# PFC-star/distributed_inference_demo

Measured on AMD Instinct MI355X. Metric: decode tokens/s, BLOOM pipeline, higher is better.
Workload: dtype bf16; 1 GPU; bloom-1b1 single stage on 1 MI355X, batch 1 decode after a 512-token prefill (BASELINE.json configs[1]); model=bloom-1b1, stages=1, batch=1, prompt=512, parallelism=pp1, weight_bytes=2130628608, weights=bf16

## Files before the change

### distributed_inference_demo_amd/build.py

```python
import hashlib
import os
import subprocess
import sys
from concurrent.futures import ThreadPoolExecutor

PKG = os.path.dirname(os.path.abspath(__file__))
ROOT = os.path.dirname(PKG)
CSRC = os.path.join(PKG, "csrc")
OBJ = os.path.join(PKG, "build")
LIB = os.path.join(PKG, "lib", "libbloomstage.so")
HIPCC = os.environ.get("HIPCC", "/opt/rocm/bin/hipcc")
ARCH = "gfx950"

SOURCES = ["kernels.hip", "attn_prefill.hip", "kv_int8.hip", "stage.hip", "codec.cpp", "safetensors.cpp"]
EXTRA = {"attn_prefill.hip": ["-mllvm", "-amdgpu-mfma-vgpr-form=1"]}
HEADERS = ["common.h", "kernels.h", "attn_merge.h", "safetensors.h"]
STAMP = os.path.join(OBJ, "build_id")
CFLAGS = ["-O3", "-std=c++17", "-fPIC", f"--offload-arch={ARCH}", "-Wall", "-Wno-unused-function",
          "-Wno-unused-variable", "-Wno-unused-result", "-Wno-unused-value", f"-I{os.path.join(ROOT, 'include')}"]


def _mtime(p):
    return os.path.getmtime(p) if os.path.exists(p) else 0.0


def source_hash() -> str:
    h = hashlib.sha256()
    for path in [os.path.join(CSRC, f) for f in SOURCES + HEADERS] + [os.path.join(ROOT, "include", "bloomstage.h")]:
        with open(path, "rb") as f:
            h.update(os.path.basename(path).encode() + b"\0" + f.read())
    return h.hexdigest()


def build(force: bool = False, verbose: bool = False) -> str:
    os.makedirs(OBJ, exist_ok=True)
    os.makedirs(os.path.dirname(LIB), exist_ok=True)
    bid = source_hash()
    old = open(STAMP).read().strip() if os.path.exists(STAMP) else ""
    restamp = old != bid
    hdr_t = max([_mtime(os.path.join(CSRC, h)) for h in HEADERS] + [_mtime(os.path.join(ROOT, "include", "bloomstage.h"))])
    jobs = []
    objs = []
    for src in SOURCES:
        sp = os.path.join(CSRC, src)
        op = os.path.join(OBJ, src + ".o")
        objs.append(op)
        if force or (restamp and src == "stage.hip") or _mtime(op) < max(_mtime(sp), hdr_t):
            flags = list(CFLAGS)
# ... 29 lines not shown
```

### distributed_inference_demo_amd/csrc/kernels.hip

```cpp
#include <array>
#include <cstdio>
#include <cstring>
#include <vector>
#include "common.h"
#include "kernels.h"
#include "attn_merge.h"

__device__ __forceinline__ __amdgpu_buffer_rsrc_t attn_rsrc(const void* p) {
  return __builtin_amdgcn_make_buffer_rsrc(const_cast<void*>(p), (short)0, (int)0xFFFFFFFF, 0x00020000);
}

#include <algorithm>
#include <cstdlib>

__device__ __forceinline__ uint64_t d_sm64(uint64_t x) {
  x += 0x9E3779B97F4A7C15ull;
  x = (x ^ (x >> 30)) * 0xBF58476D1CE4E5B9ull;
  x = (x ^ (x >> 27)) * 0x94D049BB133111EBull;
  return x ^ (x >> 31);
}
__device__ __forceinline__ uint32_t d_lb32(uint32_t x) {
  x ^= x >> 16; x *= 0x7feb352du; x ^= x >> 15; x *= 0x846ca68bu; x ^= x >> 16;
  return x;
}
// ... 120 lines not shown
  if constexpr (KIND == EPI_QKV) {
    v += to_f32(((const T*)e.bias)[n]);
    const int three = 3 * e.head_dim;
    const int head = n / three, r = n - head * three, which = r / e.head_dim, d = r - which * e.head_dim;
    if (which == 0) {
      ((T*)e.q_out)[(size_t)m * e.hidden + head * e.head_dim + d] = from_f32<T>(v);
    } else {
      const int b = m / e.seq, t = m - b * e.seq;
      const int past = e.past_dev ? e.past_dev[b] : e.past;
      const size_t idx = (((size_t)(e.slot + b) * e.n_head + head) * e.max_ctx + past + t) * e.head_dim + d;
      T* c = (T*)(which == 1 ? e.k_cache : e.v_cache);
      c[idx] = from_f32<T>(v);
    }
  } else if constexpr (KIND == EPI_RESID) {
    const size_t i = (size_t)m * e.ldo + n;
    e.out_f32[i] = (v + to_f32(((const T*)e.bias)[n])) + e.resid[i];
  } else if constexpr (KIND == EPI_GELU) {
    ((T*)e.out_act)[(size_t)m * e.ldo + n] = from_f32<T>(gelu_bloom(v + to_f32(((const T*)e.bias)[n])));
  }
}

struct EpiPre {
  uint32_t bias_bits;
  float resid;
  int past;
};

template <typename T>
__device__ __forceinline__ float bias_value(uint32_t bits) {
  if constexpr (sizeof(T) == 2) return __uint_as_float(bits << 16);
  else return __uint_as_float(bits);
}

template <typename T>
__device__ __forceinline__ EpiPre epi_prefetch(const Epi& e, int m, int n, bool valid) {
  EpiPre p{0u, 0.f, 0};
  if (e.kind == EPI_ARGMAX) return p;
  const int nn = valid ? n : 0, mm = valid ? m : 0;
  if constexpr (sizeof(T) == 2) p.bias_bits = ((const unsigned short*)e.bias)[nn];
  else p.bias_bits = ((const uint32_t*)e.bias)[nn];
  if (e.kind == EPI_RESID) p.resid = e.resid[(size_t)mm * e.ldo + nn];
  if (e.kind == EPI_QKV) p.past = e.past_dev ? e.past_dev[mm / e.seq] : e.past;
  return p;
}

template <typename T, int KIND>
__device__ __forceinline__ void epi_store_pre(const Epi& e, int m, int n, float v, const EpiPre& p) {
  if (e.col_scale) v *= e.col_scale[n];
  const float bias = bias_value<T>(p.bias_bits);
  if constexpr (KIND == EPI_QKV) {
    v += bias;
    const int three = 3 * e.head_dim;
    const int head = n / three, r = n - head * three, which = r / e.head_dim, d = r - which * e.head_dim;
    if (which == 0) {
      ((T*)e.q_out)[(size_t)m * e.hidden + head * e.head_dim + d] = from_f32<T>(v);
    } else {
      const int b = m / e.seq, t = m - b * e.seq;
      const size_t idx = (((size_t)(e.slot + b) * e.n_head + head) * e.max_ctx + p.past + t) * e.head_dim + d;
      T* c = (T*)(which == 1 ? e.k_cache : e.v_cache);
      c[idx] = from_f32<T>(v);
    }
  } else if constexpr (KIND == EPI_RESID) {
    e.out_f32[(size_t)m * e.ldo + n] = (v + bias) + p.resid;
  } else if constexpr (KIND == EPI_GELU) {
    ((T*)e.out_act)[(size_t)m * e.ldo + n] = from_f32<T>(gelu_bloom(v + bias));
  }
}

template <typename T, int K>
__device__ __forceinline__ void epi_apply(const Epi& ep, int m, int n, float v, bool valid, int ntiles) {
  if constexpr (K == EPI_ARGMAX) argmax_tile16(ep, m, n, v, valid, ntiles);
  else if (valid) epi_store<T, K>(ep, m, n, v);
}

template <int V> struct EpiKindC { static constexpr int value = V; };

template <typename F>
__device__ __forceinline__ void epi_dispatch(int kind, F&& f) {
  switch (kind) {
    case EPI_QKV: f(EpiKindC<EPI_QKV>{}); break;
    case EPI_RESID: f(EpiKindC<EPI_RESID>{}); break;
    case EPI_GELU: f(EpiKindC<EPI_GELU>{}); break;
    default: f(EpiKindC<EPI_ARGMAX>{}); break;
  }
}

struct LnArgs {
  const float* x;
  int row_stride, row_offset;
  const bf16* gamma;
  const bf16* beta;
// ... 134 lines not shown
#pragma unroll
    for (int u = 0; u < U; u++) {
      const bool live = s + u < s1;
#pragma unroll
      for (int mt = 0; mt < MT; mt++)
        acc[mt] = __builtin_amdgcn_mfma_f32_16x16x32_bf16(a[u], live ? b[mt][u] : zero8, acc[mt], 0, 0, 0);
    }
    if (more) {
#pragma unroll
      for (int u = 0; u < U; u++) a[u] = an[u];
    }
  }
  if constexpr (LN) __syncthreads();
#pragma unroll
  for (int mt = 0; mt < MT; mt++)
#pragma unroll
    for (int i = 0; i < 4; i++) red[w][mt * 16 + r][4 * g + i] = acc[mt][i];
  __syncthreads();
  const int ntiles = (N + 15) >> 4;
  epi_dispatch(ep.kind, [&](auto kc) {
    constexpr int EK = decltype(kc)::value;
    for (int t = threadIdx.x; t < MT * 256; t += WAVES * 64) {
      const int ml = t >> 4, nl = t & 15;
      float v = 0.f;
#pragma unroll
      for (int ww = 0; ww < WAVES; ww++) v += red[ww][ml][nl];
      const int n = n0 + nl;
      epi_apply<bf16, EK>(ep, ml, n, v, ml < M && n < N, ntiles);
    }
  });
}


template <int MM>
__device__ __forceinline__ void ln_rows_load(const LnArgs& ln, int M, int K, float4 (&xv)[MM][4], float (&c)[MM],
                                             uint2 (&gb)[4][2]) {
#pragma unroll
  for (int i = 0; i < 4; i++) {
    const int k = threadIdx.x * 4 + i * 1024;
    gb[i][0] = k < K ? *reinterpret_cast<const uint2*>(ln.gamma + k) : make_uint2(0u, 0u);
    gb[i][1] = k < K ? *reinterpret_cast<const uint2*>(ln.beta + k) : make_uint2(0u, 0u);
  }
#pragma unroll
  for (int m = 0; m < MM; m++) {
    const float* xr = ln.x + ((size_t)min(m, M - 1) * ln.row_stride + ln.row_offset) * K;
    c[m] = xr[0];
#pragma unroll
    for (int i = 0; i < 4; i++) {
      const int k = threadIdx.x * 4 + i * 1024;
      xv[m][i] = k < K ? *reinterpret_cast<const float4*>(xr + k) : make_float4(0.f, 0.f, 0.f, 0.f);
    }
  }
}

template <int MM>
__device__ __forceinline__ void ln_rows_finish(const LnArgs& ln, int M, int K, float4 (&xv)[MM][4],
                                               const float (&c)[MM], const uint2 (&gb)[4][2], bf16* xs,
                                               float* scratch) {
  const int lane = threadIdx.x & 63, w = threadIdx.x >> 6;
  const bool active = threadIdx.x < 256;
  float s1[MM], s2[MM];
#pragma unroll
  for (int m = 0; m < MM; m++) {
    float a1 = 0.f, a2 = 0.f;
#pragma unroll
    for (int i = 0; i < 4; i++) {
      if (threadIdx.x * 4 + i * 1024 < K) {
        const float d0 = xv[m][i].x - c[m], d1 = xv[m][i].y - c[m], d2 = xv[m][i].z - c[m], d3 = xv[m][i].w - c[m];
        a1 += (d0 + d1) + (d2 + d3);
        a2 += (d0 * d0 + d1 * d1) + (d2 * d2 + d3 * d3);
      }
    }
    s1[m] = wave_sum(a1);
    s2[m] = wave_sum(a2);
  }
  if (lane == 0 && active) {
#pragma unroll
    for (int m = 0; m < MM; m++) {
      scratch[w * 8 + m] = s1[m];
      scratch[32 + w * 8 + m] = s2[m];
    }
  }
  __syncthreads();
  float mean[MM], rstd[MM];
  const float invk = 1.0f / (float)K;
// ... 119 lines not shown
      for (int i = 0; i < 4; i++) {
        if (active && (int)threadIdx.x * 4 + i * 1024 < K) {
          if (pass == 0) a += (v[m][i].x + v[m][i].y) + (v[m][i].z + v[m][i].w);
          else {
            const float d0 = v[m][i].x - mean[m], d1 = v[m][i].y - mean[m], d2 = v[m][i].z - mean[m], d3 = v[m][i].w - mean[m];
            a += (d0 * d0 + d1 * d1) + (d2 * d2 + d3 * d3);
          }
        }
      }
      a = wave_sum(a);
      if (lane == 0 && active) scratch[pass * 32 + w * 8 + m] = a;
    }
    __syncthreads();
#pragma unroll
    for (int m = 0; m < MM; m++) {
      const float t = ((scratch[pass * 32 + m] + scratch[pass * 32 + 8 + m]) +
                       (scratch[pass * 32 + 16 + m] + scratch[pass * 32 + 24 + m])) * invk;
      if (pass == 0) mean[m] = t;
      else rstd[m] = 1.0f / sqrtf(t + eps);
    }
  }
  __syncthreads();
}

__device__ __forceinline__ void bf16x4_to_f32(const uint2 raw, float4& o) {
  o = make_float4(__uint_as_float(raw.x << 16), __uint_as_float(raw.x & 0xFFFF0000u),
                  __uint_as_float(raw.y << 16), __uint_as_float(raw.y & 0xFFFF0000u));
}

template <int MM>
__device__ __forceinline__ void emb_rows_prefetch(const LnArgs& ln, int M, int K, int (&id)[MM], uint2 (&egb)[4][2],
                                                  uint2 (&gb)[4][2]) {
#pragma unroll
  for (int m = 0; m < MM; m++) id[m] = ln.ids[min(m, M - 1)];
#pragma unroll
  for (int i = 0; i < 4; i++) {
    const int k = min((int)threadIdx.x * 4 + i * 1024, K - 4);
    egb[i][0] = *reinterpret_cast<const uint2*>(ln.emb_g + k);
    egb[i][1] = *reinterpret_cast<const uint2*>(ln.emb_b + k);
    gb[i][0] = *reinterpret_cast<const uint2*>(ln.gamma + k);
    gb[i][1] = *reinterpret_cast<const uint2*>(ln.beta + k);
  }
}

template <int MM>
__device__ __forceinline__ void emb_rows_finish(const LnArgs& ln, int M, int K, const int (&id)[MM],
                                                const uint2 (&egb)[4][2], const uint2 (&gb)[4][2], bf16* xs,
                                                float* scratch) {
  float4 v[MM][4];
#pragma unroll
  for (int m = 0; m < MM; m++) {
    const bf16* row = ln.wemb + (size_t)id[m] * K;
#pragma unroll
    for (int i = 0; i < 4; i++) {
      const int k = min((int)threadIdx.x * 4 + i * 1024, K - 4);
      bf16x4_to_f32(*reinterpret_cast<const uint2*>(row + k), v[m][i]);
    }
  }
  float mean[MM], rstd[MM];
  ln_stats_256<MM>(v, K, ln.eps, scratch, mean, rstd);
  const bool active = threadIdx.x < 256;
#pragma unroll
  for (int i = 0; i < 4; i++) {
    float4 g, b;
    bf16x4_to_f32(egb[i][0], g);
    bf16x4_to_f32(egb[i][1], b);
    const int k = (int)threadIdx.x * 4 + i * 1024;
// ... 4 lines not shown
      v[m][i].z = (v[m][i].z - mean[m]) * rstd[m] * g.z + b.z;
      v[m][i].w = (v[m][i].w - mean[m]) * rstd[m] * g.w + b.w;
      if (blockIdx.x == 0 && active && k < K && m < M) *reinterpret_cast<float4*>(ln.x_out + (size_t)m * K + k) = v[m][i];
    }
  }
  ln_stats_256<MM>(v, K, ln.eps, scratch, mean, rstd);
#pragma unroll
  for (int i = 0; i < 4; i++) {
    const int k = (int)threadIdx.x * 4 + i * 1024;
    if (active && k < K) {
      float4 g, b;
      bf16x4_to_f32(gb[i][0], g);
      bf16x4_to_f32(gb[i][1], b);
#pragma unroll
      for (int m = 0; m < MM; m++) {
        if (m < M) {
          typedef __bf16 bf16x4 __attribute__((ext_vector_type(4)));
          bf16x4 o;
          o[0] = (bf16)((v[m][i].x - mean[m]) * rstd[m] * g.x + b.x);
          o[1] = (bf16)((v[m][i].y - mean[m]) * rstd[m] * g.y + b.y);
          o[2] = (bf16)((v[m][i].z - mean[m]) * rstd[m] * g.z + b.z);
          o[3] = (bf16)((v[m][i].w - mean[m]) * rstd[m] * g.w + b.w);
          *reinterpret_cast<bf16x4*>(xs + (size_t)m * K + k) = o;
        }
      }
    }
  }
  __syncthreads();
}

template <int R, int MM, int U, int XM, int FL = 0, bool SYNC = false>
__device__ __forceinline__ void gemv_rows_block(const bf16* __restrict__ W, const bf16* __restrict__ X, const LnArgs& ln,
                                                const AttnParts& pa, int M, int N, int K, const Epi& ep, int bid,
                                                char* smem, unsigned* wait, unsigned target) {
  if constexpr (!SYNC) wait = nullptr;
  constexpr bool LN = XM == X_LN;
  BS_STAMP(0);
  float* scratch = reinterpret_cast<float*>(smem);
  bf16* xs = reinterpret_cast<bf16*>(smem + 256);
  const int lane = threadIdx.x & 63, w = threadIdx.x >> 6, nw = blockDim.x >> 6;
  const int n0 = (bid * nw + w) * R;
  const bf16* wr[R];
#pragma unroll
  for (int r = 0; r < R; r++) wr[r] = W + (size_t)min(n0 + r, N - 1) * K;
  const int er = lane / MM, em = lane % MM;
  const EpiPre pre = epi_prefetch<bf16>(ep, em, n0 + er, lane < R * MM && em < M && n0 + er < N);
  float4 xv[LN ? MM : 1][4];
  float xc[LN ? MM : 1];
  uint2 gb[4][2];
  if constexpr (LN) {
    if (threadIdx.x < 256) ln_rows_load<MM>(ln, M, K, xv, xc, gb);
  }
  int eid[XM == X_EMB ? MM : 1];
  uint2 egb[4][2];
  if constexpr (XM == X_EMB) emb_rows_prefetch<MM>(ln, M, K, eid, egb, gb);
  const int kq = K >> 2, ngroups = M * kq;
  PartsRegs pr[XM == X_PARTS ? kPartsPre : 1];
  auto pld1 = [wait](const float* p, size_t i) {
    if (wait) return __uint_as_float(__builtin_amdgcn_raw_buffer_load_b32(attn_rsrc(p), (uint32_t)(i * 4), 0, 16));
    return p[i];
  };
  auto pld4 = [wait](const float* p, size_t i) {
    if (wait)
      return __builtin_bit_cast(float4, __builtin_amdgcn_raw_buffer_load_b128(attn_rsrc(p), (uint32_t)(i * 4), 0, 16));
    return *reinterpret_cast<const float4*>(p + i);
  };
  if constexpr (XM == X_PARTS) {
    if (!wait) {
#pragma unroll
      for (int it = 0; it < kPartsPre; it++) {
        const int g = min((int)threadIdx.x + it * (int)blockDim.x, ngroups - 1);
        attn_parts_load(pa, g / kq, (g % kq) * 4, pld1, pld4, pr[it]);
      }
    }
  }
  bf16x8 wv[U][R];
#pragma unroll
  for (int u = 0; u < U; u++) {
    const int k = min(u * 512 + lane * 8, K - 8);
#pragma unroll
    for (int r = 0; r < R; r++) wv[u][r] = wload<!(FL & 1)>(wr[r] + k);
  }
  const bf16* xg;
  int xstride;
  if constexpr (LN) {
    ln_rows_finish<MM>(ln, M, K, xv, xc, gb, xs, scratch);
    xg = xs; xstride = K;
  } else if constexpr (XM == X_EMB) {
    emb_rows_finish<MM>(ln, M, K, eid, egb, gb, xs, scratch);
    xg = xs; xstride = K;
  } else if constexpr (XM == X_PARTS) {
    if (wait) {
      if (threadIdx.x == 0) {
        unsigned spins = 0;
        while (__builtin_amdgcn_raw_buffer_load_b32(attn_rsrc(wait), 0, 0, 16) < target) {
          __builtin_amdgcn_s_sleep(2);
          if (++spins > (1u << 22)) {
            __builtin_amdgcn_raw_buffer_store_b32(1u, attn_rsrc(wait), 8, 0, 16);
            break;
          }
        }
      }
      __syncthreads();
#pragma unroll
      for (int it = 0; it < kPartsPre; it++) {
        const int g = min((int)threadIdx.x + it * (int)blockDim.x, ngroups - 1);
        attn_parts_load(pa, g / kq, (g % kq) * 4, pld1, pld4, pr[it]);
      }
    }
    auto put = [&](int g, const PartsRegs& r) {
      float o[4];
      attn_parts_combine(pa.nsplit, r, o);
      typedef __bf16 bf16x4 __attribute__((ext_vector_type(4)));
      bf16x4 v;
#pragma unroll
      for (int j = 0; j < 4; j++) v[j] = (bf16)o[j];
      *reinterpret_cast<bf16x4*>(xs + (size_t)(g / kq) * K + (g % kq) * 4) = v;
    };
#pragma unroll
    for (int it = 0; it < kPartsPre; it++) {
      const int g = threadIdx.x + it * blockDim.x;
      if (g < ngroups) put(g, pr[it]);
    }
    for (int g = threadIdx.x + kPartsPre * blockDim.x; g < ngroups; g += blockDim.x) {
      PartsRegs r;
      attn_parts_load(pa, g / kq, (g % kq) * 4, pld1, pld4, r);
      put(g, r);
    }
    __syncthreads();
    xg = xs; xstride = K;
  } else {
    xg = X; xstride = K;
  }
  BS_STAMP(1);
  float acc[R][MM];
#pragma unroll
  for (int r = 0; r < R; r++)
#pragma unroll
    for (int m = 0; m < MM; m++) acc[r][m] = 0.f;
  const bf16x8 zero8 = (bf16x8){0, 0, 0, 0, 0, 0, 0, 0};
  for (int kb = 0; kb < K; kb += 512 * U) {
    if (kb) {
#pragma unroll
      for (int u = 0; u < U; u++) {
        const int k = min(kb + u * 512 + lane * 8, K - 8);
#pragma unroll
        for (int r = 0; r < R; r++) wv[u][r] = wload<!(FL & 1)>(wr[r] + k);
      }
    }
#pragma unroll
    for (int u = 0; u < U; u++) {
      const int kk = kb + u * 512 + lane * 8;
      const bool live = kk < K;
      const int k = min(kk, K - 8);
#pragma unroll
      for (int m = 0; m < MM; m++) {
        bf16x8 xv;
// ... 18 lines not shown
      if (lane == 0) {
#pragma unroll
        for (int r = 0; r < R; r++)
#pragma unroll
          for (int m = 0; m < MM; m++) tv[(w * R + r) * MM + m] = acc[r][m];
      }
      __syncthreads();
      if (threadIdx.x < 64) {
        const int col = threadIdx.x & 15, m = threadIdx.x >> 4;
        const int n = bid * 16 + col;
        const float v = m < MM ? tv[col * MM + (m < MM ? m : 0)] : 0.f;
        argmax_tile16(ep, m, n, v, m < M && n < N, (N + 15) >> 4);
      }
    } else {
      if (lane < R * MM) {
        float v = 0.f;
#pragma unroll
        for (int r = 0; r < R; r++)
#pragma unroll
          for (int m = 0; m < MM; m++) v = (lane == r * MM + m) ? acc[r][m] : v;
        const int n = n0 + er;
        if constexpr (FL & 4) {
          if (v == 12345.f) ep.keys[0] = 1;
        } else if (em < M && n < N) {
          epi_store_pre<bf16, EK>(ep, em, n, v, pre);
        }
      }
    }
  });
  BS_STAMP(3);
}

template <int R, int MM, int U, int XM, int FL = 0, int LB = 256>
__global__ __launch_bounds__(LB) void gemv_rows_kernel(const bf16* __restrict__ W, const bf16* __restrict__ X,
                                                         LnArgs ln, AttnParts pa, int M, int N, int K, Epi ep) {
  extern __shared__ __attribute__((aligned(16))) char smem[];
  gemv_rows_block<R, MM, U, XM, FL>(W, X, ln, pa, M, N, K, ep, blockIdx.x, smem, nullptr, 0u);
}

__device__ __forceinline__ void q8x16_to_bf16(const u32x4v raw, bf16x8& lo, bf16x8& hi) {
  const uint32_t v[4] = {raw.x ^ 0x80808080u, raw.y ^ 0x80808080u, raw.z ^ 0x80808080u, raw.w ^ 0x80808080u};
#pragma unroll
  for (int i = 0; i < 2; i++) {
    bf16x8& o = i ? hi : lo;
    const uint32_t a = v[2 * i], b = v[2 * i + 1];
    o[0] = (bf16)((float)(a & 0xFF) - 128.f); o[1] = (bf16)((float)((a >> 8) & 0xFF) - 128.f);
    o[2] = (bf16)((float)((a >> 16) & 0xFF) - 128.f); o[3] = (bf16)((float)(a >> 24) - 128.f);
    o[4] = (bf16)((float)(b & 0xFF) - 128.f); o[5] = (bf16)((float)((b >> 8) & 0xFF) - 128.f);
    o[6] = (bf16)((float)((b >> 16) & 0xFF) - 128.f); o[7] = (bf16)((float)(b >> 24) - 128.f);
  }
}

template <int T, int MT, int WAVES>
__device__ __forceinline__ void tiles_epilogue(const f32x4 (&acc)[T][MT], float* red, int M, int N, int n0,
                                               const Epi& ep) {
  constexpr int RS = MT * 16 + 1;
  const int lane = threadIdx.x & 63, w = threadIdx.x >> 6;
  const int r = lane & 15, g = lane >> 4;
  const int KS = gridDim.y, ks = blockIdx.y;
  float* rw = red + (size_t)w * (T * 16) * RS;
#pragma unroll
  for (int t = 0; t < T; t++)
#pragma unroll
    for (int mt = 0; mt < MT; mt++)
#pragma unroll
      for (int i = 0; i < 4; i++) rw[(t * 16 + 4 * g + i) * RS + mt * 16 + r] = acc[t][mt][i];
  __syncthreads();
  const int ntiles = (N + 15) >> 4;
  constexpr int TOTAL = T * 16 * MT * 16, NTH = WAVES * 64;
  constexpr int ITER = (TOTAL + NTH - 1) / NTH;
// ... 1133 lines not shown
    Ws[ty][tx] = wr[k0 + tx];
    __syncthreads();
#pragma unroll
    for (int kk = 0; kk < 16; kk++) acc += Xs[ty][kk] * Ws[tx][kk];
    __syncthreads();
  }
  const int m = m0 + ty, n = n0 + tx;
  epi_dispatch(ep.kind, [&](auto kc) {
    epi_apply<float, decltype(kc)::value>(ep, m, n, acc, m < M && n < N, (N + 15) >> 4);
  });
}

template <int WAVES, int MT, bool LN>
static void gemv_launch(const bf16* X, const LnArgs& ln, const bf16* W, int M, int N, int K, const Epi& ep,
                        hipStream_t s) {
  size_t shm = sizeof(float) * WAVES * MT * 16 * 17;
  if (LN) shm += (size_t)M * K * sizeof(bf16);
  gemv_mfma_kernel<WAVES, MT, 4, LN, 0, 0><<<(N + 15) / 16, WAVES * 64, shm, s>>>(W, X, ln, M, N, K, ep);
}

static int gemv_waves(int N, int K) {
  const int ntiles = (N + 15) / 16, ksteps = K / 32;
  int waves = 4;
  while (waves < 16 && ntiles * waves < 2048 && waves * 2 <= ksteps) waves *= 2;
  return waves;
}

template <int R, int MM, int XM, int U = 2, int FL = 0>
static void gemv_rows_launch(const bf16* X, const LnArgs& ln, const AttnParts& pa, const bf16* W, int M, int N,
                             int K, const Epi& ep, hipStream_t s, int waves = 4) {
  const size_t shm = 256 + (XM != X_PLAIN ? (size_t)M * K * sizeof(bf16) : 0);
  const int blocks = (N + waves * R - 1) / (waves * R);
  if (waves <= 4) {
    gemv_rows_kernel<R, MM, U, XM, FL, 256><<<blocks, waves * 64, shm, s>>>(W, X, ln, pa, M, N, K, ep);
  } else if constexpr (MM <= 2) {
    gemv_rows_kernel<R, MM, U, XM, FL, 1024><<<blocks, waves * 64, shm, s>>>(W, X, ln, pa, M, N, K, ep);
  }
}

static void rows_geometry(int N, int K, int M, int r_default, int* R, int* waves) {
  if (M > 2) { *R = r_default; *waves = 4; return; }
  const int rows_cu = (N + 255) / 256;
  int r = K <= 2048 ? 2 : 1;
  while ((rows_cu + r - 1) / r > 16 && r < 4) r *= 2;
  if ((rows_cu + r - 1) / r < 4) r = 1;
  *R = r;
  *waves = std::max(4, std::min(16, (rows_cu + r - 1) / r));
}

static void rows_plan(int XM, int M, int N, int K, int* R, int* waves, int* U) {
  const bool LN = XM == X_LN || XM == X_EMB;
  const int R0 = !LN ? (K <= 2048 ? 2 : 1) : (N >= 12288 ? 4 : (N >= 2048 ? 2 : 1));
  rows_geometry(N, K, M, R0, R, waves);
  const int cpr = K / 512;
  int u = (K % 512) ? 4 : (cpr <= 3 || cpr == 5 || cpr == 8 || cpr == 12) ? cpr
        : (cpr % 12 == 0 ? 12 : (cpr % 8 == 0 ? 8 : (cpr % 5 == 0 ? 5 : 4)));
  if (*waves > 4) {
    const int cap = (XM == X_PLAIN ? 12 : 8) / (M == 1 ? 1 : 2);
    while (*R * u > cap) u = (u % 2 == 0) ? u / 2 : (u > 4 ? 4 : u - 1);
  }
  *U = u;
}

template <int XM>
static bool gemv_rows_dispatch(const bf16* x, const LnArgs& ln, const AttnParts& pa, const bf16* w, int M, int N,
                               int K, const Epi& ep, hipStream_t s) {
  if (M > 4 || (K % 8) != 0 || K < 8 || (XM != X_PLAIN && K > 4096)) return false;
  if ((XM == X_PLAIN || XM == X_LN) && ep.kind != EPI_ARGMAX && tiles_take(M, K) && (K % 64) == 0) return false;
  if (XM == X_PLAIN && M > 2 && ep.kind != EPI_ARGMAX && (size_t)N * K > (size_t)16 << 20) return false;
// ... 810 lines not shown
            for (int i = 0; i < 4; i++) {
              xf[i] = f2{__uint_as_float(a0[i] << 16), __uint_as_float(a0[i] & 0xFFFF0000u)};
              xf[4 + i] = f2{__uint_as_float(a1[i] << 16), __uint_as_float(a1[i] & 0xFFFF0000u)};
            }
#pragma unroll
            for (int i = 0; i < 8; i++) xs[m] += xf[i];
#pragma unroll
            for (int r = 0; r < R; r++)
#pragma unroll
              for (int i = 0; i < 8; i++) acc[r][m] = __builtin_elementwise_fma(xf[i], wf[r][i], acc[r][m]);
          }
        }
      }
    }
  }
  float mine = 0.f;
#pragma unroll
  for (int r = 0; r < R; r++)
#pragma unroll
    for (int m = 0; m < MM; m++) {
      if (m < M) {
        const float t = wave_sum((acc[r][m].x + acc[r][m].y) - 128.f * (xs[m].x + xs[m].y));
        if (lane == r * MM + m) mine = t;
      }
    }
  const int r = lane / MM, m = lane - r * MM;
  if (lane < R * MM && m < M && n0 + r < N) epi_store<bf16, KIND>(ep, m, n0 + r, mine);
}

template <int R, int MM, bool LN, int CW, bool XL = false, int UQ = 2, bool PARTS = false, bool WIDE = false>
__global__ __launch_bounds__(WIDE ? 1024 : 256) void gemv_q8_kernel(const int8_t* __restrict__ Q, const float* __restrict__ scale,
                                                      const bf16* __restrict__ X, LnArgs ln, AttnParts pa, int M,
                                                      int N, int K, Epi ep) {
  epi_dispatch(ep.kind, [&](auto kc) {
    if constexpr (decltype(kc)::value != EPI_ARGMAX)
      gemv_q8_body<R, MM, LN, decltype(kc)::value, CW, XL, UQ, PARTS>(Q, scale, X, ln, pa, M, N, K, ep);
  });
}

template <int R, int MM, bool LN = false, bool PARTS = false>
static void gemv_q8_launch(const int8_t* Q, const float* scale, const bf16* X, const LnArgs& ln, int M, int N, int K,
                           const Epi& ep, hipStream_t s, const AttnParts& pa = AttnParts{}) {
  const size_t shm = (LN || PARTS) ? (size_t)M * K * sizeof(bf16) : 0;
  const int blocks = (N + 4 * R - 1) / (4 * R);
  const int steps = (K + 1023) / 1024;
  const int uq = (size_t)N * K > (12u << 20) ? 1 : min(steps <= 2 ? 2 : steps <= 4 ? 4 : steps <= 6 ? 6 : 8, R >= 4 ? 4 : 8);
  const bool wide_xl = (size_t)M * K * sizeof(bf16) <= 65536;
  if constexpr (MM == 1 && R <= 2) {
    int rr = 0, waves = 0;
    rows_geometry(N, K, M, R, &rr, &waves);
    if ((size_t)N * K <= (32u << 20) && rr <= 2 && waves >= 4 && uq <= 6) {
      auto go = [&](auto rc) {
        constexpr int RW = decltype(rc)::value;
        const int wb = (N + waves * RW - 1) / (waves * RW);
        const dim3 g(wb), t(waves * 64);
        if constexpr (!LN && !PARTS) {
          if (wide_xl) {
            const size_t shx = (size_t)M * K * sizeof(bf16);
            if (uq == 1) gemv_q8_kernel<RW, 1, false, 16, true, 1, false, true><<<g, t, shx, s>>>(Q, scale, X, ln, pa, M, N, K, ep);
            else if (uq <= 2) gemv_q8_kernel<RW, 1, false, 16, true, 2, false, true><<<g, t, shx, s>>>(Q, scale, X, ln, pa, M, N, K, ep);
            else if (uq <= 4) gemv_q8_kernel<RW, 1, false, 16, true, 4, false, true><<<g, t, shx, s>>>(Q, scale, X, ln, pa, M, N, K, ep);
            else gemv_q8_kernel<RW, 1, false, 16, true, 6, false, true><<<g, t, shx, s>>>(Q, scale, X, ln, pa, M, N, K, ep);
            return;
          }
        }
        if (uq == 1) gemv_q8_kernel<RW, 1, LN, 16, false, 1, PARTS, true><<<g, t, shm, s>>>(Q, scale, X, ln, pa, M, N, K, ep);
// ... 120 lines not shown
template <int MM, int U, int R>
__global__ __launch_bounds__(1024) void gemv_head_screen_kernel(const int8_t* __restrict__ Q, const float* __restrict__ scale,
                                                           const float* __restrict__ cb, LnArgs ln, int M, int ntiles,
                                                           int K, float2* __restrict__ hilo, float* __restrict__ rnorm) {
  typedef float f2 __attribute__((ext_vector_type(2)));
  extern __shared__ __attribute__((aligned(16))) char smem[];
  float* scratch = reinterpret_cast<float*>(smem);
  bf16* xs = reinterpret_cast<bf16*>(smem + 256);
  const int lane = threadIdx.x & 63, nw = blockDim.x >> 6;
  const int w = __builtin_amdgcn_readfirstlane(threadIdx.x >> 6);
  const int t0 = (int)((long long)blockIdx.x * ntiles / gridDim.x);
  const int t1 = (int)((long long)(blockIdx.x + 1) * ntiles / gridDim.x);
  constexpr int G = 16 / R;
  const int steps = (K + 512 * U - 1) / (512 * U), gs = G * steps;
  const int nunits = max((t1 - t0 - w + nw - 1) / nw, 0) * gs;
  typedef unsigned int u32x2v __attribute__((ext_vector_type(2)));
  struct Buf { u32x2v wv[U][R]; float sc[R], cc[R]; };
  auto issue = [&](int i, Buf& b) {
    const int ti = i / gs, rem = i - ti * gs, g = rem / steps, kb = rem - g * steps;
    const int n0 = (t0 + w + ti * nw) * 16 + g * R;
#pragma unroll
    for (int u = 0; u < U; u++) {
      const int col = min((kb * U + u) * 512 + lane * 8, K - 8);
#pragma unroll
      for (int r = 0; r < R; r++)
        b.wv[u][r] = __builtin_nontemporal_load(reinterpret_cast<const u32x2v*>(Q + (size_t)(n0 + r) * K + col));
    }
#pragma unroll
    for (int r = 0; r < R; r++) { b.sc[r] = scale[n0 + r]; b.cc[r] = cb[n0 + r]; }
  };
  float4 xv[MM][4];
  float xc[MM];
  uint2 gb[4][2];
  if (threadIdx.x < 256) ln_rows_load<MM>(ln, M, K, xv, xc, gb);
  Buf b0{}, b1{}, b2{};
  if (nunits > 0) issue(0, b0);
  if (nunits > 1) issue(1, b1);
  if (threadIdx.x < 8) xs[(size_t)M * K + threadIdx.x] = (bf16)0.f;
  ln_rows_finish<MM>(ln, M, K, xv, xc, gb, xs, scratch);
  float rm[MM];
#pragma unroll
  for (int m = 0; m < MM; m++) {
    float a = 0.f;
    for (int k = lane * 8; k < K; k += 512) {
      float v[8];
      load8(xs + (size_t)min(m, M - 1) * K + k, v);
#pragma unroll
      for (int j = 0; j < 8; j++) a = fmaf(v[j], v[j], a);
    }
    rm[m] = sqrtf(wave_sum(a)) * (1.0f + 0x1p-10f);
    if (blockIdx.x == 0 && threadIdx.x == 0 && m < M) rnorm[m] = rm[m];
    rm[m] *= 1.0f + 0x1p-20f;
  }
  float hi[MM], lo[MM], chk[MM];
  f2 acc[R][MM];
#pragma unroll
  for (int m = 0; m < MM; m++) {
    hi[m] = -INFINITY; lo[m] = -INFINITY; chk[m] = 0.f;
#pragma unroll
    for (int r = 0; r < R; r++) acc[r][m] = f2{0.f, 0.f};
  }
  auto compute = [&](int i, const Buf& cur) {
    const int ti = i / gs, rem = i - ti * gs, g = rem / steps, kb = rem - g * steps;
#pragma unroll
    for (int u = 0; u < U; u++) {
      const int kk = (kb * U + u) * 512 + lane * 8;
      f2 xf[MM][4];
// ... 83 lines not shown
  }
  L = wave_max(L);
  bad = __any(bad);
  if ((threadIdx.x & 63) == 0) { shl[threadIdx.x >> 6] = L; shb[threadIdx.x >> 6] = bad; }
  if (threadIdx.x == 0) cnt = 0;
  __syncthreads();
  L = shl[0]; bad = shb[0];
  for (int j = 1; j < 16; j++) { L = fmaxf(L, shl[j]); bad |= shb[j]; }
  bool all = bad || !(fabsf(L) < INFINITY) || !(fabsf(r) < INFINITY);
  if (!all) {
    if (fits) {
#pragma unroll
      for (int j = 0; j < kSelPer; j++) {
        const int i = threadIdx.x + j * 1024;
        if (i < ntiles && v[j].x >= L) li[atomicAdd(&cnt, 1)] = i;
      }
    } else {
      for (int i = threadIdx.x; i < ntiles; i += 1024)
        if (hl[i].x >= L) li[atomicAdd(&cnt, 1)] = i;
    }
    __syncthreads();
    all = cnt == 0;
  }
  if (all)
    for (int i = threadIdx.x; i < ntiles; i += 1024) li[i] = i;
  if (threadIdx.x == 0) { count[m] = all ? ntiles : cnt; lstar[m] = L; }
}

template <int MM, int U>
__global__ __launch_bounds__(256) void head_rescore_kernel(const bf16* __restrict__ W, LnArgs ln, int M, int N, int K,
                                                           Epi ep, const int* __restrict__ list,
                                                           const int* __restrict__ count, int ntiles) {
  extern __shared__ __attribute__((aligned(16))) char smem[];
  bool first = true;
  for (int m = 0; m < M; m++) {
    const int c = min(max(count[m], 0), ntiles);
    for (int i = blockIdx.x; i < c; i += gridDim.x) {
      const int tile = min(max(list[(size_t)m * ntiles + i], 0), ntiles - 1);
      if (!first) __syncthreads();
      first = false;
      gemv_rows_block<4, MM, U, X_LN>(W, nullptr, ln, AttnParts{}, M, N, K, ep, tile, smem, nullptr, 0u);
    }
  }
}

__global__ __launch_bounds__(1024) void head_screen_finalize_kernel(const unsigned long long* __restrict__ keys, int ntiles,
                                                                    const int* __restrict__ list,
                                                                    const int* __restrict__ count, int* tokens,
                                                                    int* past_adv, int seq) {
  __shared__ unsigned long long sh[17];
  const int m = blockIdx.x;
  const int c = min(max(count[m], 0), ntiles);
  unsigned long long best = 0;
  for (int i = threadIdx.x; i < c; i += 1024) {
    const int tile = min(max(list[(size_t)m * ntiles + i], 0), ntiles - 1);
    const unsigned long long k = keys[(size_t)m * ntiles + tile];
    best = k > best ? k : best;
  }
  best = block_max_u64(best, sh);
  if (threadIdx.x == 0) {
    if (tokens) tokens[m] = (int)(0xFFFFFFFFu - (uint32_t)(best & 0xFFFFFFFFull));
    if (past_adv) past_adv[m] += seq;
  }
}

bool head_screen_supported(int M, int K) { return M >= 1 && M <= 2 && K % 32 == 0 && K >= 32 && K <= 4096; }

template <int MM>
static void head_screen_launch(const HeadScreen& hs, const LnArgs& ln, int M, int ntiles, int K, int grid, hipStream_t s) {
  const size_t shm = 256 + (size_t)M * K * sizeof(bf16) + 16;
  float2* hl = reinterpret_cast<float2*>(hs.hilo);
  const int cpr = (K + 511) / 512;
#define HS_GO(UU, RR) gemv_head_screen_kernel<MM, UU, RR><<<grid, 1024, shm, s>>>(hs.Q, hs.scale, hs.cb, ln, M, ntiles, K, hl, hs.rnorm)
  if (cpr == 1) HS_GO(1, 4);
// ... 35 lines not shown
```

Baseline: 1224 tokens/s.

## Preload kernel arguments into SGPRs and reorder early loads in GEMV kernels

Enables kernarg preloading for kernels.hip and moves the most-used scalar arguments (LN pointers, strides, wave count) to the front of the gemv_rows kernel signature. Inline-asm pins force those values into SGPRs early. A lane_zero trick turns uniform scalar loads into vector loads so they issue alongside the other global loads, and the gamma/beta loads are reordered. The aim is to cut kernel-prologue latency in the small per-token decode kernels, at the cost of fragile asm constraints and compiler-flag dependence.

```diff
diff --git a/distributed_inference_demo_amd/build.py b/distributed_inference_demo_amd/build.py
--- a/distributed_inference_demo_amd/build.py
+++ b/distributed_inference_demo_amd/build.py
@@ -13,7 +13,8 @@
 ARCH = "gfx950"
 
 SOURCES = ["kernels.hip", "attn_prefill.hip", "kv_int8.hip", "stage.hip", "codec.cpp", "safetensors.cpp"]
-EXTRA = {"attn_prefill.hip": ["-mllvm", "-amdgpu-mfma-vgpr-form=1"]}
+EXTRA = {"attn_prefill.hip": ["-mllvm", "-amdgpu-mfma-vgpr-form=1"],
+         "kernels.hip": ["-mllvm", "-amdgpu-kernarg-preload-count=16"]}
 HEADERS = ["common.h", "kernels.h", "attn_merge.h", "safetensors.h"]
 STAMP = os.path.join(OBJ, "build_id")
 CFLAGS = ["-O3", "-std=c++17", "-fPIC", f"--offload-arch={ARCH}", "-Wall", "-Wno-unused-function",
diff --git a/distributed_inference_demo_amd/csrc/kernels.hip b/distributed_inference_demo_amd/csrc/kernels.hip
--- a/distributed_inference_demo_amd/csrc/kernels.hip
+++ b/distributed_inference_demo_amd/csrc/kernels.hip
@@ -176,6 +176,17 @@
   else return __uint_as_float(bits);
 }
 
+__device__ __forceinline__ int lane_zero() {
+  int z;
+  asm("v_mov_b32 %0, 0" : "=v"(z));
+  return z;
+}
+
+template <typename T>
+__device__ __forceinline__ void kernarg_pin1(T v) { asm volatile("" ::"s"(v)); }
+template <typename... T>
+__device__ __forceinline__ void kernarg_pin(T... v) { (kernarg_pin1(v), ...); }
+
 template <typename T>
 __device__ __forceinline__ EpiPre epi_prefetch(const Epi& e, int m, int n, bool valid) {
   EpiPre p{0u, 0.f, 0};
@@ -184,7 +195,7 @@
   if constexpr (sizeof(T) == 2) p.bias_bits = ((const unsigned short*)e.bias)[nn];
   else p.bias_bits = ((const uint32_t*)e.bias)[nn];
   if (e.kind == EPI_RESID) p.resid = e.resid[(size_t)mm * e.ldo + nn];
-  if (e.kind == EPI_QKV) p.past = e.past_dev ? e.past_dev[mm / e.seq] : e.past;
+  if (e.kind == EPI_QKV && e.past_dev) p.past = e.past_dev[mm / e.seq + lane_zero()];
   return p;
 }
 
@@ -200,7 +211,8 @@
       ((T*)e.q_out)[(size_t)m * e.hidden + head * e.head_dim + d] = from_f32<T>(v);
     } else {
       const int b = m / e.seq, t = m - b * e.seq;
-      const size_t idx = (((size_t)(e.slot + b) * e.n_head + head) * e.max_ctx + p.past + t) * e.head_dim + d;
+      const unsigned past = e.past_dev ? (unsigned)p.past : (unsigned)e.past;
+      const size_t idx = (((size_t)(e.slot + b) * e.n_head + head) * e.max_ctx + past + t) * e.head_dim + d;
       T* c = (T*)(which == 1 ? e.k_cache : e.v_cache);
       c[idx] = from_f32<T>(v);
     }
@@ -401,25 +413,30 @@
 }
 
 
-template <int MM>
+template <int MM, bool VSHIFT = true>
 __device__ __forceinline__ void ln_rows_load(const LnArgs& ln, int M, int K, float4 (&xv)[MM][4], float (&c)[MM],
                                              uint2 (&gb)[4][2]) {
-#pragma unroll
-  for (int i = 0; i < 4; i++) {
-    const int k = threadIdx.x * 4 + i * 1024;
-    gb[i][0] = k < K ? *reinterpret_cast<const uint2*>(ln.gamma + k) : make_uint2(0u, 0u);
-    gb[i][1] = k < K ? *reinterpret_cast<const uint2*>(ln.beta + k) : make_uint2(0u, 0u);
-  }
+  auto gamma_beta = [&] {
+#pragma unroll
+    for (int i = 0; i < 4; i++) {
+      const int k = threadIdx.x * 4 + i * 1024;
+      gb[i][0] = k < K ? *reinterpret_cast<const uint2*>(ln.gamma + k) : make_uint2(0u, 0u);
+      gb[i][1] = k < K ? *reinterpret_cast<const uint2*>(ln.beta + k) : make_uint2(0u, 0u);
+    }
+  };
+  if constexpr (!VSHIFT) gamma_beta();
 #pragma unroll
   for (int m = 0; m < MM; m++) {
     const float* xr = ln.x + ((size_t)min(m, M - 1) * ln.row_stride + ln.row_offset) * K;
-    c[m] = xr[0];
+    if constexpr (!VSHIFT) c[m] = xr[0];
 #pragma unroll
     for (int i = 0; i < 4; i++) {
       const int k = threadIdx.x * 4 + i * 1024;
       xv[m][i] = k < K ? *reinterpret_cast<const float4*>(xr + k) : make_float4(0.f, 0.f, 0.f, 0.f);
     }
-  }
+    if constexpr (VSHIFT) c[m] = xr[lane_zero()];
+  }
+  if constexpr (VSHIFT) gamma_beta();
 }
 
 template <int MM>
@@ -605,7 +622,7 @@
 __device__ __forceinline__ void emb_rows_prefetch(const LnArgs& ln, int M, int K, int (&id)[MM], uint2 (&egb)[4][2],
                                                   uint2 (&gb)[4][2]) {
 #pragma unroll
-  for (int m = 0; m < MM; m++) id[m] = ln.ids[min(m, M - 1)];
+  for (int m = 0; m < MM; m++) id[m] = ln.ids[min(m, M - 1) + lane_zero()];
 #pragma unroll
   for (int i = 0; i < 4; i++) {
     const int k = min((int)threadIdx.x * 4 + i * 1024, K - 4);
@@ -676,25 +693,29 @@
 template <int R, int MM, int U, int XM, int FL = 0, bool SYNC = false>
 __device__ __forceinline__ void gemv_rows_block(const bf16* __restrict__ W, const bf16* __restrict__ X, const LnArgs& ln,
                                                 const AttnParts& pa, int M, int N, int K, const Epi& ep, int bid,
-                                                char* smem, unsigned* wait, unsigned target) {
+                                                int nw, char* smem, unsigned* wait, unsigned target) {
   if constexpr (!SYNC) wait = nullptr;
   constexpr bool LN = XM == X_LN;
   BS_STAMP(0);
   float* scratch = reinterpret_cast<float*>(smem);
   bf16* xs = reinterpret_cast<bf16*>(smem + 256);
-  const int lane = threadIdx.x & 63, w = threadIdx.x >> 6, nw = blockDim.x >> 6;
+  const int lane = threadIdx.x & 63, w = threadIdx.x >> 6, nthreads = nw * 64;
   const int n0 = (bid * nw + w) * R;
   const bf16* wr[R];
 #pragma unroll
   for (int r = 0; r < R; r++) wr[r] = W + (size_t)min(n0 + r, N - 1) * K;
-  const int er = lane / MM, em = lane % MM;
-  const EpiPre pre = epi_prefetch<bf16>(ep, em, n0 + er, lane < R * MM && em < M && n0 + er < N);
   float4 xv[LN ? MM : 1][4];
   float xc[LN ? MM : 1];
   uint2 gb[4][2];
   if constexpr (LN) {
     if (threadIdx.x < 256) ln_rows_load<MM>(ln, M, K, xv, xc, gb);
   }
+  asm volatile("" ::: "memory");
+  kernarg_pin(ep.kind, ep.bias, ep.resid, ep.ldo, ep.seq, ep.past_dev, ep.past);
+  if constexpr (XM == X_EMB) kernarg_pin(ln.ids, ln.emb_g, ln.emb_b);
+  if constexpr (XM == X_PARTS) kernarg_pin(pa.acc, pa.ml, pa.nsplit, pa.n_head, pa.head_dim, pa.max_chunks, pa.slot);
+  const int er = lane / MM, em = lane % MM;
+  const EpiPre pre = epi_prefetch<bf16>(ep, em, n0 + er, lane < R * MM && em < M && n0 + er < N);
   int eid[XM == X_EMB ? MM : 1];
   uint2 egb[4][2];
   if constexpr (XM == X_EMB) emb_rows_prefetch<MM>(ln, M, K, eid, egb, gb);
@@ -713,7 +734,7 @@
     if (!wait) {
 #pragma unroll
       for (int it = 0; it < kPartsPre; it++) {
-        const int g = min((int)threadIdx.x + it * (int)blockDim.x, ngroups - 1);
+        const int g = min((int)threadIdx.x + it * nthreads, ngroups - 1);
         attn_parts_load(pa, g / kq, (g % kq) * 4, pld1, pld4, pr[it]);
       }
     }
@@ -748,7 +769,7 @@
       __syncthreads();
 #pragma unroll
       for (int it = 0; it < kPartsPre; it++) {
-        const int g = min((int)threadIdx.x + it * (int)blockDim.x, ngroups - 1);
+        const int g = min((int)threadIdx.x + it * nthreads, ngroups - 1);
         attn_parts_load(pa, g / kq, (g % kq) * 4, pld1, pld4, pr[it]);
       }
     }
@@ -763,10 +784,10 @@
     };
 #pragma unroll
     for (int it = 0; it < kPartsPre; it++) {
-      const int g = threadIdx.x + it * blockDim.x;
+      const int g = threadIdx.x + it * nthreads;
       if (g < ngroups) put(g, pr[it]);
     }
-    for (int g = threadIdx.x + kPartsPre * blockDim.x; g < ngroups; g += blockDim.x) {
+    for (int g = threadIdx.x + kPartsPre * nthreads; g < ngroups; g += nthreads) {
       PartsRegs r;
       attn_parts_load(pa, g / kq, (g % kq) * 4, pld1, pld4, r);
       put(g, r);
@@ -851,10 +872,14 @@
 }
 
 template <int R, int MM, int U, int XM, int FL = 0, int LB = 256>
-__global__ __launch_bounds__(LB) void gemv_rows_kernel(const bf16* __restrict__ W, const bf16* __restrict__ X,
-                                                         LnArgs ln, AttnParts pa, int M, int N, int K, Epi ep) {
+__global__ __launch_bounds__(LB) void gemv_rows_kernel(const bf16* __restrict__ W, const bf16* __restrict__ X, int M,
+                                                         int N, int K, int nw, const float* __restrict__ lnx,
+                                                         int ln_stride, int ln_offset, const bf16* __restrict__ lng,
+                                                         const bf16* __restrict__ lnb, LnArgs ln, AttnParts pa,
+                                                         Epi ep) {
   extern __shared__ __attribute__((aligned(16))) char smem[];
-  gemv_rows_block<R, MM, U, XM, FL>(W, X, ln, pa, M, N, K, ep, blockIdx.x, smem, nullptr, 0u);
+  ln.x = lnx; ln.row_stride = ln_stride; ln.row_offset = ln_offset; ln.gamma = lng; ln.beta = lnb;
+  gemv_rows_block<R, MM, U, XM, FL>(W, X, ln, pa, M, N, K, ep, blockIdx.x, nw, smem, nullptr, 0u);
 }
 
 __device__ __forceinline__ void q8x16_to_bf16(const u32x4v raw, bf16x8& lo, bf16x8& hi) {
@@ -2054,9 +2079,11 @@
   const size_t shm = 256 + (XM != X_PLAIN ? (size_t)M * K * sizeof(bf16) : 0);
   const int blocks = (N + waves * R - 1) / (waves * R);
   if (waves <= 4) {
-    gemv_rows_kernel<R, MM, U, XM, FL, 256><<<blocks, waves * 64, shm, s>>>(W, X, ln, pa, M, N, K, ep);
+    gemv_rows_kernel<R, MM, U, XM, FL, 256><<<blocks, waves * 64, shm, s>>>(
+        W, X, M, N, K, waves, ln.x, ln.row_stride, ln.row_offset, ln.gamma, ln.beta, ln, pa, ep);
   } else if constexpr (MM <= 2) {
-    gemv_rows_kernel<R, MM, U, XM, FL, 1024><<<blocks, waves * 64, shm, s>>>(W, X, ln, pa, M, N, K, ep);
+    gemv_rows_kernel<R, MM, U, XM, FL, 1024><<<blocks, waves * 64, shm, s>>>(
+        W, X, M, N, K, waves, ln.x, ln.row_stride, ln.row_offset, ln.gamma, ln.beta, ln, pa, ep);
   }
 }
 
@@ -2933,6 +2960,10 @@
 __global__ __launch_bounds__(WIDE ? 1024 : 256) void gemv_q8_kernel(const int8_t* __restrict__ Q, const float* __restrict__ scale,
                                                       const bf16* __restrict__ X, LnArgs ln, AttnParts pa, int M,
                                                       int N, int K, Epi ep) {
+  kernarg_pin(Q, M, N, K, ep.kind, (int)blockDim.x);
+  if constexpr (LN) kernarg_pin(ln.x, ln.row_stride, ln.row_offset, ln.gamma, ln.beta);
+  else if constexpr (PARTS) kernarg_pin(pa.acc, pa.ml, pa.nsplit, pa.n_head, pa.head_dim, pa.max_chunks, pa.slot);
+  else kernarg_pin(X);
   epi_dispatch(ep.kind, [&](auto kc) {
     if constexpr (decltype(kc)::value != EPI_ARGMAX)
       gemv_q8_body<R, MM, LN, decltype(kc)::value, CW, XL, UQ, PARTS>(Q, scale, X, ln, pa, M, N, K, ep);
@@ -3119,7 +3150,7 @@
   float4 xv[MM][4];
   float xc[MM];
   uint2 gb[4][2];
-  if (threadIdx.x < 256) ln_rows_load<MM>(ln, M, K, xv, xc, gb);
+  if (threadIdx.x < 256) ln_rows_load<MM, false>(ln, M, K, xv, xc, gb);
   Buf b0{}, b1{}, b2{};
   if (nunits > 0) issue(0, b0);
   if (nunits > 1) issue(1, b1);
@@ -3269,6 +3300,8 @@
                                                            Epi ep, const int* __restrict__ list,
                                                            const int* __restrict__ count, int ntiles) {
   extern __shared__ __attribute__((aligned(16))) char smem[];
+  kernarg_pin(W, ln.x, ln.row_stride, ln.row_offset, ln.gamma, ln.beta, M, N, K, ep.kind, list, count, ntiles,
+              (int)gridDim.x);
   bool first = true;
   for (int m = 0; m < M; m++) {
     const int c = min(max(count[m], 0), ntiles);
@@ -3276,7 +3309,7 @@
       const int tile = min(max(list[(size_t)m * ntiles + i], 0), ntiles - 1);
       if (!first) __syncthreads();
       first = false;
-      gemv_rows_block<4, MM, U, X_LN>(W, nullptr, ln, AttnParts{}, M, N, K, ep, tile, smem, nullptr, 0u);
+      gemv_rows_block<4, MM, U, X_LN>(W, nullptr, ln, AttnParts{}, M, N, K, ep, tile, 4, smem, nullptr, 0u);
     }
   }
 }
```

Measured after the change: 1233 tokens/s, median of 6. About the same (+0.7%).
